# mathjeff/Mapper

Measured on NVIDIA B200. Metric: aligned reads/sec, higher is better.
Workload: dtype f64

## Files before the change

mapper_b200/csrc/xm_align.h:

```cpp
#pragma once
#include "xm_seed.h"

namespace xm {

struct Blk { int a_start, b_start, a_len, b_len; };
struct DAln {
  int valid, n;
  Blk* b;
  double penalty, aligned;
  int ref_reversed;
};
struct ACtx {
  SeqView a; int a_reversed_obj;
  SeqView b;
};
struct Sec { int start, end; XM_INLINE int length() const { return end - start; } };

struct MatcherD {
  int ref_start, ref_len, block_len, section_len, max_section_index;
  int loc_size;
  uint32_t* materialized;
  int mat_words;
  int16_t* tables; int table_entries, n_slots, slots_used;
  int slot_section[8];
};
static const int16_t T_NO = -1, T_MULTI = -2;
struct Analysis {
  MatcherD* matcher;
  int predicted, last_checked, confident;
  double max_ins, max_del;
};

XM_INLINE DAln aln_null() { DAln a; a.valid = 0; a.n = 0; a.b = nullptr; a.penalty = 0; a.aligned = 0; a.ref_reversed = 0; return a; }

XM_FN double block_penalty(const Params& p, const ACtx& c, const Blk& k) {
  double pen = 0;
  if (k.a_len == k.b_len) {
#if defined(__CUDA_ARCH__)
    const int lane = (int)(threadIdx.x & 31);
    XM_NOUNROLL
    for (int base = 0; base < k.a_len; base += 32) {
      const int i = base + lane;
      double v = 0;
      if (i < k.a_len) v = p.base_penalty(c.a.at(k.a_start + i), c.b.at(k.b_start + i));
      unsigned m = __ballot_sync(0xffffffffu, v != 0);
      XM_NOUNROLL
      while (m) { const int src = __ffs(m) - 1; m &= m - 1; pen += __shfl_sync(0xffffffffu, v, src); }
    }
    __syncwarp();
#else
    XM_NOUNROLL
    for (int i = 0; i < k.a_len; i++) pen += p.base_penalty(c.a.at(k.a_start + i), c.b.at(k.b_start + i));
#endif
  } else if (k.a_len > 0) { pen += p.ins_start; pen += p.ins_ext * k.a_len; }
  else { pen += p.del_start; pen += p.del_ext * k.b_len; }
  return pen;
}
XM_FN double block_penalty_range(const Params& p, const SeqView& a, const SeqView& b, const Blk& k, int start_b, int end_b) {
  double pen = 0;
  if (k.a_len == k.b_len) {
#if defined(__CUDA_ARCH__)
    const int lane = (int)(threadIdx.x & 31);
    XM_NOUNROLL
    for (int base = 0; base < k.a_len; base += 32) {
      const int i = base + lane, bi = k.b_start + i;
      double v = 0;
      if (i < k.a_len && bi >= start_b && bi < end_b) v = p.base_penalty(a.at(k.a_start + i), b.at(bi));
      unsigned m = __ballot_sync(0xffffffffu, v != 0);
      XM_NOUNROLL
      while (m) { const int src = __ffs(m) - 1; m &= m - 1; pen += __shfl_sync(0xffffffffu, v, src); }
    }
    __syncwarp();
#else
    XM_NOUNROLL
    for (int i = 0; i < k.a_len; i++) { int bi = k.b_start + i; if (bi >= start_b && bi < end_b) pen += p.base_penalty(a.at(k.a_start + i), b.at(bi)); }
#endif
  } else if (k.b_start < end_b && k.b_start + k.b_len > start_b) {
    if (k.a_len > 0) { pen += p.ins_start; pen += p.ins_ext * k.a_len; } else { pen += p.del_start; pen += p.del_ext * k.b_len; }
  }
  return pen;
}
XM_FN DAln new_aln(const Params& p, const ACtx& c, Blk* blocks, int n, int ref_reversed) {
  int aligned_len = 0;
  double total = 0;
  XM_NOUNROLL
  for (int i = 0; i < n; i++) { total += block_penalty(p, c, blocks[i]); aligned_len += blocks[i].a_len; }
  if (n > 0 && p.start_free && blocks[0].b_len == 0) total -= p.ins_start;
  double aligned = total;
  if (n > 0) { int un = c.a.len - aligned_len; total += (double)un * p.unaligned; }
  DAln r; r.valid = 1; r.n = n; r.b = blocks; r.penalty = total; r.aligned = aligned; r.ref_reversed = ref_reversed;
  return r;
}
XM_INLINE int aln_start_a(const DAln& a) { return a.b[0].a_start; }
XM_INLINE int aln_end_a(const DAln& a) { return a.b[a.n - 1].a_start + a.b[a.n - 1].a_len; }
XM_INLINE int aln_start_b(const DAln& a) { return a.b[0].b_start; }
XM_INLINE int aln_end_b(const DAln& a) { return a.b[a.n - 1].b_start + a.b[a.n - 1].b_len; }

static const int M_NO = -1, M_MULTI = -2, M_UNKNOWN = -3;

XM_HD inline int log4_floor_plus1(int x) {
  int k = 0; long long p = 4;
  XM_NOUNROLL
  while (p <= (long long)x) { k++; p *= 4; }
  return k + 1;
}
XM_FN MatcherD* matcher_new(WS& w, const ACtx& c, const Sec& rsec, int section_len) {
  MatcherD* m = (MatcherD*)w.salloc(sizeof(MatcherD));
  if (!m) return nullptr;
  if (section_len < 1) section_len = 1;
  m->block_len = log4_floor_plus1(section_len * 5);
  if (m->block_len < 3) m->block_len = 3;
  m->ref_start = rsec.start; m->ref_len = rsec.length(); m->section_len = section_len;
  m->max_section_index = (c.b.len - 1 - m->ref_start) / section_len;
  m->loc_size = 0;
  int n_sec = imin(m->max_section_index + 1, (m->ref_len + 1) / section_len + 2);
  int words = (n_sec + 31) / 32;
  if (words < 1) words = 1;
  if (words > 4096) words = 4096;
  m->mat_words = words;
  m->materialized = (uint32_t*)w.salloc((long long)words * 4);
  if (!m->materialized) return nullptr;
  XM_NOUNROLL
  for (int i = 0; i < words; i++) m->materialized[i] = 0;
  m->tables = nullptr; m->table_entries = 0; m->n_slots = 0; m->slots_used = 0;
  if (section_len >= 3 && section_len < 32000 && m->block_len <= 7) {
    int entries = 1 << (2 * m->block_len);
    int slots = imin(8, m->max_section_index + 1);
    long long bytes = (long long)slots * entries * 2 + 16;
    if (slots > 0 && w.scratch_top + bytes + 4096 <= w.scratch_size / 2) {
      char* p = (char*)w.salloc(bytes);
      p += (16 - ((uintptr_t)p & 15)) & 15;
      m->tables = (int16_t*)p; m->table_entries = entries; m->n_slots = slots;
    }
  }
  return m;
}
XM_HD inline int matcher_encode(const SeqView& s, int index, int block_len) {
  if (index + block_len > s.len) return M_UNKNOWN;
  int sum = 0;
  XM_NOUNROLL
  for (int i = 0; i < block_len; i++) {
    uint8_t h = s.at(index + i);
    if (bp_is_ambiguous(h)) return M_UNKNOWN;
    sum = sum * 4 + (h == 1 ? 0 : h == 2 ? 1 : h == 4 ? 2 : 3);
  }
  return sum;
}
template <class F>
XM_INLINE void matcher_scan_encodings(const MatcherD& m, const SeqView& ref, int section_index, F&& f) {
  int max_poss = (1 << (2 * m.block_len)) - 1;
  int prev = M_UNKNOWN;
  int start = m.ref_start + section_index * m.section_len;
  int end = imin(start + m.section_len, m.ref_start + m.ref_len - m.block_len);
  XM_NOUNROLL
  for (int i = start; i < end; i++) {
    int enc;
    if (prev == M_UNKNOWN) enc = matcher_encode(ref, i, m.block_len);
    else {
      uint8_t nc = ref.at(i + m.block_len - 1);
      if (bp_is_ambiguous(nc)) enc = M_UNKNOWN;
      else enc = ((prev * 4) & max_poss) + (nc == 1 ? 0 : nc == 2 ? 1 : nc == 4 ? 2 : 3);
    }
    if (enc == M_UNKNOWN) continue;
    f(i - start, enc);
    prev = enc;
  }
}
XM_FN int matcher_section_value(WS& w, MatcherD& m, const SeqView& ref, int section_index, int target) {
  XM_CHECK_MASK(w);
  int start = m.ref_start + section_index * m.section_len;
  if (m.tables != nullptr) {
    int slot = -1;
    XM_NOUNROLL
    for (int i = 0; i < m.slots_used; i++) if (m.slot_section[i] == section_index) { slot = i; break; }
    if (slot < 0 && m.slots_used < m.n_slots) {
      PhaseClock pc_(&w.st_cyc[4]);
      slot = m.slots_used++;
      m.slot_section[slot] = section_index;
      int16_t* t = m.tables + (long long)slot * m.table_entries;
#if defined(__CUDA_ARCH__)
      {
        uint4 fill = make_uint4(0xFFFFFFFFu, 0xFFFFFFFFu, 0xFFFFFFFFu, 0xFFFFFFFFu);
        uint4* t4 = (uint4*)t;
        int n16 = m.table_entries / 8;
        XM_NOUNROLL
        for (int i = (int)(threadIdx.x & 31); i < n16; i += 32) t4[i] = fill;
        __syncwarp();
      }
#else
      XM_NOUNROLL
      for (int i = 0; i < m.table_entries; i++) t[i] = T_NO;
#endif
      matcher_scan_encodings(m, ref, section_index, [&](int rel, int enc) { t[enc] = (t[enc] == T_NO) ? (int16_t)rel : T_MULTI; });
    }
    if (slot >= 0) {
      int16_t v = m.tables[(long long)slot * m.table_entries + target];
      return v == T_NO ? M_NO : v == T_MULTI ? M_MULTI : start + (int)v;
    }
  }
  int value = M_NO;
  matcher_scan_encodings(m, ref, section_index, [&](int rel, int enc) { if (enc == target) value = (value == M_NO) ? start + rel : M_MULTI; });
  return value;
}
XM_HD inline bool matcher_get_section(WS& w, MatcherD& m, int index) {
  if (index >= m.mat_words * 32) { w.fail(Q_NEED_MORE); return false; }
  if (m.loc_size > index) return (m.materialized[index >> 5] >> (index & 31)) & 1;
  m.loc_size = index + 1;
  m.materialized[index >> 5] |= (1u << (index & 31));
  return true;
}
XM_FN int matcher_scan_section(const MatcherD& m, const ACtx& c, int query_index, int section_index) {
  int result = M_NO;
  int start = m.ref_start + section_index * m.section_len, end = start + m.section_len;
  XM_NOUNROLL
  for (int i = start; i < end; i++) {
    bool ok = !(i + m.block_len > m.ref_start + m.ref_len);
    XM_NOUNROLL
    for (int k = 0; ok && k < m.block_len; k++) {
      if (query_index + k >= c.a.len || i + k >= c.b.len) { ok = false; break; }
      if (!bp_can_match(c.a.at(query_index + k), c.b.at(i + k))) ok = false;
    }
    if (ok) { if (result == M_NO) result = i; else return M_MULTI; }
  }
  return result;
}
XM_FN int matcher_lookup(WS& w, MatcherD& m, const ACtx& c, int query_index, int min_ref, int max_ref) {
  XM_CHECK_MASK(w);
  if (min_ref < 0) return M_UNKNOWN;
  if (max_ref > c.b.len) return M_UNKNOWN;
  int enc = matcher_encode(c.a, query_index, m.block_len);
  if (enc < 0) return M_UNKNOWN;
  int matched = M_NO;
  int min_sec = imax(0, (min_ref - m.ref_start) / m.section_len);
  int max_sec = imin(m.max_section_index, (max_ref - m.ref_start) / m.section_len);
  XM_NOUNROLL
  for (int si = min_sec; si <= max_sec; si++) {
    bool have = matcher_get_section(w, m, si);
    if (w.status != 0) return M_UNKNOWN;
    int looked;
    if (m.section_len < 3) looked = matcher_scan_section(m, c, query_index, si);
    else { if (have) looked = matcher_section_value(w, m, c.b, si, enc); else return M_UNKNOWN; }
    if (looked == M_UNKNOWN) return M_UNKNOWN;
    if (looked == M_MULTI) return M_MULTI;
    if (looked == M_NO) continue;
    if (looked < min_ref || looked > max_ref) continue;
    if (matched != M_NO) return M_MULTI;
    matched = looked;
  }
  return matched;
}

struct alignas(16) PNode { double pen, ins_x, ins_y; uint32_t stamp; uint32_t meta; };
struct alignas(8) PMeta { uint32_t stamp, meta; };
struct PEnt { uint32_t xy; int32_t next; };
struct PathState {
  Params prm; ACtx ctx;
  int an_confident; double an_max_ins, an_max_del;
  int start_a, end_a, start_b, end_b, A, B, W, H;
  int diagonal, step, reverse, may_extend;
  int start_x, start_y, goal_x, goal_y;
  PNode* nodes; uint32_t gen; uint32_t clock;
  const uint8_t* qa; const uint8_t* rb;
  PEnt* ent; int ent_cap;
  double max_interesting;
};
XM_INLINE uint8_t pa_qa(const PathState& s, int i) { return s.qa[i]; }
XM_INLINE uint8_t pa_rb(const PathState& s, int j) { return s.rb[j]; }
XM_INLINE bool pa_can_remove(const Blk& b) {
  if (b.a_len <= 0 && b.b_len <= 0) return true;
  if ((b.a_start <= 0 && b.a_len <= 0) || (b.b_start <= 0 && b.b_len <= 0)) return true;
  return false;
}
XM_INLINE uint32_t pa_pack_xy(int x, int y) { return ((uint32_t)(uint16_t)(int16_t)x << 16) | (uint32_t)(uint16_t)(int16_t)y; }

struct PaOverflow { double key; int head, tail; };
struct PaQueue {
  PEnt* ent; int n_ent, cap, free_head;
  double cur_key; int cur_head, cur_tail;
  PaOverflow* ovf; int ovf_lo, ovf_hi, cap_ovf;
#if defined(__CUDA_ARCH__)
  double bkey; int bhead, btail;
#else
  double bkey[32]; int bhead[32], btail[32];
#endif
  XM_INLINE void init(PEnt* e, int capacity, PaOverflow* o, int cap_o) {
    ent = e; n_ent = 0; cap = capacity; free_head = -1; cur_key = 0; cur_head = -1; cur_tail = -1; ovf = o; ovf_lo = 0; ovf_hi = 0; cap_ovf = cap_o;
#if defined(__CUDA_ARCH__)
    bkey = 0; bhead = -1; btail = -1;
#else
    for (int i = 0; i < 32; i++) { bkey[i] = 0; bhead[i] = -1; btail[i] = -1; }
#endif
  }
  XM_INLINE int push(double pri, int x, int y) {
    int id;
    if (n_ent < cap) id = n_ent++;
    else { if (free_head < 0) return 1; id = free_head; free_head = ent[id].next; }
    PEnt e; e.xy = pa_pack_xy(x, y); e.next = -1;
    ent[id] = e;
    if (pri == cur_key) {
      if (cur_tail >= 0) ent[cur_tail].next = id; else cur_head = id;
      cur_tail = id;
      return 0;
    }
#if defined(__CUDA_ARCH__)
    const int lane = (int)(threadIdx.x & 31);
    const unsigned hit = __ballot_sync(0xffffffffu, bhead >= 0 && bkey == pri);
    if (hit != 0) {
      const int b = __ffs(hit) - 1;
      const int t = __shfl_sync(0xffffffffu, btail, b);
      ent[t].next = id;
      if (lane == b) btail = id;
      return 0;
    }
#else
    for (int b = 0; b < 32; b++) if (bhead[b] >= 0 && bkey[b] == pri) { ent[btail[b]].next = id; btail[b] = id; return 0; }
#endif
    int lo = ovf_lo, hi = ovf_hi;
#if defined(__CUDA_ARCH__)
    XM_NOUNROLL
    while (hi - lo > 0) {
      const int n = hi - lo;
      const int stride = (n + 31) >> 5;
      const int at = lo + imin(n, (lane + 1) * stride) - 1;
      const bool less = ovf[at].key < pri;
      const int k = __popc(__ballot_sync(0xffffffffu, less));
      const int nlo = lo + imin(n, k * stride);
      if (k >= 32 || nlo >= hi) { lo = hi; break; }
      hi = lo + imin(n, (k + 1) * stride); lo = nlo;
      if (stride == 1) { break; }
    }
#else
    XM_NOUNROLL
    while (lo < hi) { const int mid = (lo + hi) >> 1; if (ovf[mid].key < pri) lo = mid + 1; else hi = mid; }
#endif
    if (lo < ovf_hi && ovf[lo].key == pri) { ent[ovf[lo].tail].next = id; ovf[lo].tail = id; return 0; }
#if defined(__CUDA_ARCH__)
    const unsigned fre = __ballot_sync(0xffffffffu, bhead < 0);
    if (fre != 0) { const int b = __ffs(fre) - 1; if (lane == b) { bkey = pri; bhead = id; btail = id; } return 0; }
#else
    for (int b = 0; b < 32; b++) if (bhead[b] < 0) { bkey[b] = pri; bhead[b] = id; btail[b] = id; return 0; }
#endif
    if (ovf_hi >= cap_ovf) {
      if (ovf_lo == 0) return 2;
      const int n = ovf_hi - ovf_lo;
#if defined(__CUDA_ARCH__)
      XM_NOUNROLL
      for (int base = 0; base < n; base += 32) {
        const int i = base + lane;
        PaOverflow t; if (i < n) t = ovf[ovf_lo + i];
        __syncwarp();
        if (i < n) ovf[i] = t;
        __syncwarp();
      }
#else
      for (int i = 0; i < n; i++) ovf[i] = ovf[ovf_lo + i];
#endif
      lo -= ovf_lo; ovf_lo = 0; ovf_hi = n;
    }
    {
#if defined(__CUDA_ARCH__)
      XM_NOUNROLL
      for (int top = ovf_hi; top > lo; top -= 32) {
        const int i = top - 1 - lane;
        PaOverflow t; if (i >= lo) t = ovf[i];
        __syncwarp();
        if (i >= lo) ovf[i + 1] = t;
        __syncwarp();
      }
#else
      for (int i = ovf_hi - 1; i >= lo; i--) ovf[i + 1] = ovf[i];
#endif
      PaOverflow t; t.key = pri; t.head = id; t.tail = id;
      ovf[lo] = t;
      ovf_hi++;
    }
    return 0;
  }
  XM_INLINE bool pop(int& x, int& y) {
    if (cur_head < 0) {
      bool have = false; double best = 0; int where = -1;
#if defined(__CUDA_ARCH__)
      const int lane = (int)(threadIdx.x & 31);
      const unsigned live = __ballot_sync(0xffffffffu, bhead >= 0);
      if (live != 0) {
        const unsigned long long bits = (unsigned long long)__double_as_longlong(bkey);
        const unsigned hi = bhead >= 0 ? (unsigned)(bits >> 32) : 0xffffffffu;
        const unsigned mhi = __reduce_min_sync(0xffffffffu, hi);
        const unsigned lo = (bhead >= 0 && hi == mhi) ? (unsigned)bits : 0xffffffffu;
        const unsigned mlo = __reduce_min_sync(0xffffffffu, lo);
        const unsigned who = __ballot_sync(0xffffffffu, bhead >= 0 && hi == mhi && (unsigned)bits == mlo);
        where = __ffs(who) - 1;
        best = __longlong_as_double((long long)(((unsigned long long)mhi << 32) | mlo));
        have = true;
      }
#else
      for (int b = 0; b < 32; b++) if (bhead[b] >= 0 && (!have || bkey[b] < best)) { have = true; best = bkey[b]; where = b; }
#endif
      if (ovf_lo < ovf_hi && (!have || ovf[ovf_lo].key < best)) { have = true; best = ovf[ovf_lo].key; where = 32; }
      if (!have) return false;
      cur_key = best;
      if (where >= 32) { cur_head = ovf[ovf_lo].head; cur_tail = ovf[ovf_lo].tail; ovf_lo++; if (ovf_lo == ovf_hi) { ovf_lo = 0; ovf_hi = 0; } }
      else {
#if defined(__CUDA_ARCH__)
        cur_head = __shfl_sync(0xffffffffu, bhead, where); cur_tail = __shfl_sync(0xffffffffu, btail, where);
        if (lane == where) bhead = -1;
#else
        cur_head = bhead[where]; cur_tail = btail[where]; bhead[where] = -1;
#endif
      }
    }
    const PEnt e = ent[cur_head];
    ent[cur_head].next = free_head; free_head = cur_head;
    cur_head = e.next;
    if (cur_head < 0) cur_tail = -1;
    x = (int)(int16_t)(e.xy >> 16); y = (int)(int16_t)(e.xy & 0xffffu);
    return true;
  }
};

XM_INLINE int pa_signed_dist(const PathState& s, int x, int y) { return x - y - s.diagonal; }
XM_INLINE PNode pa_node(const PathState& s, int idx) {
#if defined(__CUDA_ARCH__)
  const double2 a = __ldcg((const double2*)&s.nodes[idx]);
  const double2 b = __ldcg((const double2*)&s.nodes[idx] + 1);
  PNode n; n.pen = a.x; n.ins_x = a.y; n.ins_y = b.x;
  const unsigned long long m = (unsigned long long)__double_as_longlong(b.y);
  n.stamp = (uint32_t)m; n.meta = (uint32_t)(m >> 32);
  return n;
#else
  return s.nodes[idx];
#endif
}
XM_INLINE bool pa_get(const PathState& s, int x, int y, int& idx) {
  if (x < 0 || x >= s.W || y < 0 || y >= s.H) return false;
  idx = x * s.H + y;
  return (pa_node(s, idx).meta >> 8) == s.gen;
}
XM_HD inline double pa_estimate(const PathState& s, int x, int y, const PNode& n, int fl) {
  if (!s.an_confident) return n.pen;
  int sd = pa_signed_dist(s, x, y);
  const Params& p = s.prm;
  if (fl & 2) {
    if (sd * s.step > 0) { double ie = fabs(sd * p.ins_ext); if (ie > s.an_max_ins) return XM_DISALLOWED; }
    else { double de = fabs(sd * p.del_ext); if (de > s.an_max_del) return XM_DISALLOWED; }
    if (fl & 4) return n.pen;
    return n.pen + dmin(p.ins_start + p.ins_ext, p.del_start + p.del_ext);
  }
  if (sd * s.step < 0) {
    double ie = fabs(sd * p.ins_ext);
    if (ie > s.an_max_ins) return XM_DISALLOWED;
    double is = dmin(p.ins_start, n.ins_x - n.pen);
    return n.pen + is + ie;
  } else {
    double de = fabs(sd * p.del_ext);
    if (de > s.an_max_del) return XM_DISALLOWED;
    double ds = dmin(p.del_start, n.ins_y - n.pen);
    return n.pen + ds + de;
  }
}
XM_FN int pa_search(WS& w, PathState& S, PaOverflow* ovf, int cap_ovf, int& last_x, int& last_y) {
  XM_CHECK_MASK(w);
  const int A = S.A, B = S.B, H = S.H, step = S.step, goal_x = S.goal_x, goal_y = S.goal_y, diag = S.diagonal;
  const bool may_extend = S.may_extend != 0, confident = S.an_confident != 0;
  const double ins_start = S.prm.ins_start, ins_ext = S.prm.ins_ext, del_start = S.prm.del_start, del_ext = S.prm.del_ext, unaligned = S.prm.unaligned;
  const double max_ins = S.an_max_ins, max_del = S.an_max_del, budget = S.max_interesting + 0.000001;
  const double min_indel = dmin(ins_start + ins_ext, del_start + del_ext);
  const double* pen_tab = S.prm.pen_tab; const uint8_t* cls_tab = S.prm.cls_tab;
  PNode* nodes = S.nodes; const uint8_t* qa = S.qa; const uint8_t* rb = S.rb;
  const uint32_t gen = S.gen; const int W = S.W;
  uint32_t clock = S.clock;
  PaQueue Q;
  Q.init(S.ent, S.ent_cap, ovf, cap_ovf);
  int qrc = 0;
  {
    const int start_x = S.start_x, start_y = S.start_y;
    const bool along_y = B >= A;
    double sisp = XM_DISALLOWED;
    if (along_y && may_extend) sisp = S.prm.starting_ins_start();
    const int cnt1 = (along_y ? imax(0, B - A) : imax(0, A - B)) + 1;
    const int cnt2 = may_extend ? imax(0, j2i(S.an_max_ins / del_ext) - 1) : 0;
    XM_NOUNROLL
    for (int i = 0; i < cnt1 + cnt2 && qrc == 0; i++) {
      PNode n; int x, y;
      if (i < cnt1) {
        n.pen = 0; n.ins_x = along_y ? sisp : XM_DISALLOWED; n.ins_y = XM_DISALLOWED;
        x = along_y ? start_x : start_x + i * step; y = along_y ? start_y + i * step : start_y;
      } else {
        const int k = i - cnt1 + 1;
        x = start_x + k * step; y = start_y;
        n.pen = k * unaligned; n.ins_x = XM_DISALLOWED; n.ins_y = XM_DISALLOWED;
        if (x < -32000 || x > 32000) { qrc = 1; break; }
      }
      n.stamp = ++clock; n.meta = gen << 8;
      qrc = Q.push(pa_estimate(S, x, y, n, 0), x, y);
      if (x >= 0 && x < W) nodes[x * H + y] = n;
    }
  }
  unsigned long long steps = 0;
  int rc = 2;
  XM_NOUNROLL
  while (qrc == 0) {
    int tx, ty;
    if (!Q.pop(tx, ty)) { w.fail(Q_INTERNAL); break; }
    const double active = Q.cur_key;
    steps++;
    if (active > budget) { rc = 1; break; }
    if (tx == goal_x) { last_x = tx; last_y = ty; rc = 0; break; }
    XM_NOUNROLL
    for (int nb = 0; nb < 3; nb++) {
      const int x = tx + (nb != 1 ? step : 0), y = ty + (nb != 0 ? step : 0);
      if (x <= 0 || x > A || y <= 0 || y > B) continue;
      const int ie = x * H + y, il = ie - step * H, iu = ie - step, id = il - step;
      const PMeta me = *(const PMeta*)&nodes[ie].stamp, ml = *(const PMeta*)&nodes[il].stamp, mu = *(const PMeta*)&nodes[iu].stamp, md = *(const PMeta*)&nodes[id].stamp;
      const bool he = (me.meta >> 8) == gen, hl = (ml.meta >> 8) == gen, hu = (mu.meta >> 8) == gen, hd = (md.meta >> 8) == gen;
      if (he) {
        uint32_t newest = 0;
        if (hl && ml.stamp > newest) newest = ml.stamp;
        if (hu && mu.stamp > newest) newest = mu.stamp;
        if (hd && md.stamp > newest) newest = md.stamp;
        if (me.stamp > newest) continue;
      }
      const uint32_t fl_ = hl ? (1u | (ml.meta & 6u)) : 0u, fu = hu ? (1u | (mu.meta & 6u)) : 0u, fd = hd ? (1u | (md.meta & 6u)) : 0u;
      double ins_x = XM_DISALLOWED, ins_y = XM_DISALLOWED, overlay = XM_DISALLOWED;
      if (hd) overlay = nodes[id].pen + pen_tab[((int)qa[x - 1] << 4) | (int)rb[y - 1]];
      if (hl) {
        const double lp = nodes[il].pen;
        if (y == goal_y && may_extend) ins_x = lp + unaligned;
        else {
          bool allowed = (cls_tab[((int)qa[x - 1 - step] << 5) | (int)rb[y - 1]] & 1) != 0;
          if (allowed) allowed = (cls_tab[((int)qa[x - 1] << 5) | (int)rb[y - 1 + step]] & 6) == 0;
          const double nw = allowed ? lp + ins_start + ins_ext : XM_DISALLOWED;
          ins_x = dmin(nodes[il].ins_x + ins_ext, nw);
        }
      }
      if (hu) {
        bool allowed = (cls_tab[((int)qa[x - 1] << 5) | (int)rb[y - 1 - step]] & 1) != 0;
        if (allowed) allowed = (cls_tab[((int)qa[x - 1 + step] << 5) | (int)rb[y - 1]] & 6) == 0;
        const double nw = allowed ? nodes[iu].pen + del_start + del_ext : XM_DISALLOWED;
        ins_y = dmin(nodes[iu].ins_y + del_ext, nw);
      }
      const double best = dmin(dmin(overlay, ins_x), ins_y);
      if (he && !(best < nodes[ie].pen || ins_x < nodes[ie].ins_x || ins_y < nodes[ie].ins_y)) continue;
      const int sd = x - y - diag;
      int fl = 0;
      if (best != XM_DISALLOWED) {
        const int src = (best == overlay) ? fd : (best == ins_x) ? fl_ : fu;
        fl = (src & 6) | (sd == 0 ? 2 : 4);
      }
      double est = best;
      if (confident) {
        const int sds = sd * step;
        if (fl & 2) {
          const bool over = (sds > 0) ? (fabs(sd * ins_ext) > max_ins) : (fabs(sd * del_ext) > max_del);
          if (over) est = XM_DISALLOWED;
          else if (!(fl & 4)) est = best + min_indel;
        } else if (sds < 0) {
          const double ie_ = fabs(sd * ins_ext);
          if (ie_ > max_ins) est = XM_DISALLOWED;
          else est = best + dmin(ins_start, ins_x - best) + ie_;
        } else {
          const double de = fabs(sd * del_ext);
          if (de > max_del) est = XM_DISALLOWED;
          else est = best + dmin(del_start, ins_y - best) + de;
        }
      }
      if (est < active) est = active;
      qrc = Q.push(est, x, y);
      if (qrc != 0) break;
      PNode n; n.pen = best; n.ins_x = ins_x; n.ins_y = ins_y; n.stamp = ++clock; n.meta = (gen << 8) | (uint32_t)fl;
      nodes[ie] = n;
    }
  }
  S.clock = clock;
  if (qrc != 0) { w.fail(Q_NEED_MORE); rc = 2; }
  w.st_path_steps += steps;
  return rc;
}

XM_FN DAln path_align(WS& w, const ACtx& c, const Sec& q, const Sec& r, const Params& p, Analysis& an) {
  XM_CHECK_MASK(w);
  PhaseClock pc_(&w.st_cyc[3]);
  long long mark = w.scratch_top;
  PathState* sp = (PathState*)w.salloc(sizeof(PathState));
  if (!sp) return aln_null();
  PathState& s = *sp;
  s.prm = p; s.ctx = c; s.an_confident = an.confident; s.an_max_ins = an.max_ins; s.an_max_del = an.max_del;
  s.max_interesting = q.length() * p.max_error_rate;
  s.start_a = q.start; s.end_a = q.end; s.start_b = r.start; s.end_b = r.end;
  s.A = q.length(); s.B = r.length(); s.W = s.A + 2; s.H = s.B + 2;
  s.diagonal = s.start_b - (s.start_a + an.predicted);
  {
    uint8_t* qa = (uint8_t*)w.salloc(s.A + 5); uint8_t* rb = (uint8_t*)w.salloc(s.B + 5);
    if (w.status != 0) { w.scratch_top = mark; return aln_null(); }
    qa += 2; rb += 2;
    XM_NOUNROLL
    for (int k = 0; k < 2; k++) { qa[-1 - k] = 16; qa[s.A + k] = 16; rb[-1 - k] = 16; rb[s.B + k] = 16; }
#if defined(__CUDA_ARCH__)
    for (int k = (int)(threadIdx.x & 31); k < s.A; k += 32) qa[k] = c.a.at(s.start_a + k);
    for (int k = (int)(threadIdx.x & 31); k < s.B; k += 32) rb[k] = c.b.at(s.start_b + k);
    __syncwarp();
#else
    for (int k = 0; k < s.A; k++) qa[k] = c.a.at(s.start_a + k);
    for (int k = 0; k < s.B; k++) rb[k] = c.b.at(s.start_b + k);
#endif
    s.qa = qa; s.rb = rb;
  }
  w.st_path_calls++; w.st_path_cells += (unsigned long long)s.A * (unsigned long long)s.B;
  {
    int sum_mis = 0, num_mis = 0, sum_mat = 0, num_mat = 0;
    int si = imax(s.start_a, s.start_b - an.predicted), ei = imin(s.end_a, s.end_b - an.predicted);
    int length = ei - si;
#if defined(__CUDA_ARCH__)
    XM_NOUNROLL
    for (int i = (int)(threadIdx.x & 31); i < length; i += 32) {
      int j = i - s.diagonal;
      if (j >= 0 && j < s.B) {
        if (!bp_can_match(pa_qa(s, i), pa_rb(s, j))) { sum_mis += i; num_mis++; } else { sum_mat += i; num_mat++; }
      }
    }
    __syncwarp();
    sum_mis = __reduce_add_sync(0xffffffffu, sum_mis); num_mis = __reduce_add_sync(0xffffffffu, num_mis);
    sum_mat = __reduce_add_sync(0xffffffffu, sum_mat); num_mat = __reduce_add_sync(0xffffffffu, num_mat);
#else
    XM_NOUNROLL
    for (int i = 0; i < length; i++) {
      int j = i - s.diagonal;
      if (j >= 0 && j < s.B) {
        if (!bp_can_match(pa_qa(s, i), pa_rb(s, j))) { sum_mis += i; num_mis++; } else { sum_mat += i; num_mat++; }
      }
    }
#endif
    s.reverse = (num_mis > 1 && num_mat > 1) ? ((sum_mis / num_mis) > (sum_mat / num_mat) ? 1 : 0) : 1;
  }
  if (s.reverse) { s.step = -1; s.may_extend = (s.start_b == 0); } else { s.step = 1; s.may_extend = (s.end_b == c.b.len); }
  if (s.reverse) { s.start_x = s.W - 1; s.start_y = s.H - 1; s.goal_x = 1; s.goal_y = 1; }
  else { s.start_x = 0; s.start_y = 0; s.goal_x = s.W - 2; s.goal_y = s.H - 2; }
  long long cells = (long long)s.W * (long long)s.H;
  if (s.W > 32000 || s.H > 32000) { w.fail(Q_NEED_MORE); w.scratch_top = mark; return aln_null(); }
  const long long map_words = cells * (long long)(sizeof(PNode) / 4);
  if (w.cell_hdr == nullptr || map_words > w.cell_words) { w.fail(Q_NEED_MORE); w.scratch_top = mark; return aln_null(); }
  {
    uint32_t gen = w.cell_hdr[0];
    if (gen == 0 || gen >= 0xFFFFFF) {
      const long long n16 = (w.cell_words + 3) >> 2;
#if defined(__CUDA_ARCH__)
      uint4* c4 = (uint4*)w.cellmap;
      XM_NOUNROLL
      for (long long i = (long long)(threadIdx.x & 31); i < n16; i += 32) c4[i] = make_uint4(0u, 0u, 0u, 0u);
      __syncwarp();
#else
      for (long long i = 0; i < w.cell_words; i++) w.cellmap[i] = 0;
#endif
      gen = 0;
    }
    gen++;
#if defined(__CUDA_ARCH__)
    if ((threadIdx.x & 31) == 0) w.cell_hdr[0] = gen;
    __syncwarp();
#else
    w.cell_hdr[0] = gen;
#endif
    s.nodes = (PNode*)w.cellmap; s.gen = gen; s.clock = 0;
  }
  long long remaining = w.scratch_size - w.scratch_top;
  int cap_ovf = (int)(s.max_interesting * 64.0) + 256;
  if ((long long)cap_ovf * (long long)sizeof(PaOverflow) > remaining / 8) cap_ovf = (int)((remaining / 8) / (long long)sizeof(PaOverflow));
  PaOverflow* ovf = (PaOverflow*)w.salloc((long long)cap_ovf * (long long)sizeof(PaOverflow));
  long long ent_cap = (remaining / 2) / (long long)sizeof(PEnt);
  if (ent_cap > 3 * cells + 64) ent_cap = 3 * cells + 64;
  s.ent_cap = (int)ent_cap;
  s.ent = (PEnt*)w.salloc(ent_cap * (long long)sizeof(PEnt));
  if (w.status != 0 || s.ent_cap < 8) { w.fail(Q_NEED_MORE); w.scratch_top = mark; return aln_null(); }
  int last_x = -1, last_y = -1;
  {
    const int rc = pa_search(w, s, ovf, cap_ovf, last_x, last_y);
    if (rc == 1 && w.status == 0) { w.scratch_top = mark; return aln_null(); }
  }
  if (w.status != 0) { w.scratch_top = mark; return aln_null(); }
  int max_blocks = s.A + s.B + 4;
  Blk* tb = (Blk*)w.salloc((long long)max_blocks * (long long)sizeof(Blk));
  if (!tb) { w.scratch_top = mark; return aln_null(); }
  int nb = 0;
  int i = last_x, j = last_y, idx;
  XM_NOUNROLL
  while (i != s.start_x && j != s.start_y) {
    if (!pa_get(s, i, j, idx)) { w.fail(Q_INTERNAL); break; }
    PNode node = pa_node(s, idx);
    Blk k;
    if (node.pen == node.ins_x) {
      int old_i = i;
      i -= s.step;
      XM_NOUNROLL
      while (i != s.start_x) {
        if (!pa_get(s, i, j, idx)) { w.fail(Q_INTERNAL); break; }
        const PNode o = pa_node(s, idx);
        if (o.pen + p.ins_start + p.ins_ext < o.ins_x + p.ins_ext) break;
        i -= s.step;
      }
      if (s.reverse) { k.a_start = s.start_a + old_i - 1; k.b_start = s.start_b + j - 1; k.a_len = i - old_i; k.b_len = 0; }
      else { k.a_start = s.start_a + i; k.b_start = s.start_b + j; k.a_len = old_i - i; k.b_len = 0; }
    } else if (node.pen == node.ins_y) {
      int old_j = j;
      j -= s.step;
      XM_NOUNROLL
      while (j != s.start_y) {
        if (!pa_get(s, i, j, idx)) { w.fail(Q_INTERNAL); break; }
        const PNode o = pa_node(s, idx);
        if (o.pen + p.del_start + p.del_ext < o.ins_y + p.del_ext) break;
        j -= s.step;
      }
      if (s.reverse) { k.a_start = s.start_a + i - 1; k.b_start = s.start_b + old_j - 1; k.a_len = 0; k.b_len = j - old_j; }
      else { k.a_start = s.start_a + i; k.b_start = s.start_b + j; k.a_len = 0; k.b_len = old_j - j; }
    } else {
      int old_i = i, old_j = j;
      i -= s.step; j -= s.step;
      XM_NOUNROLL
      while (i != s.start_x && j != s.start_y) {
        if (!pa_get(s, i, j, idx)) { w.fail(Q_INTERNAL); break; }
        const PNode o = pa_node(s, idx);
        if (o.pen == o.ins_x || o.pen == o.ins_y) break;
        i -= s.step; j -= s.step;
      }
      if (s.reverse) { k.a_start = s.start_a + old_i - 1; k.b_start = s.start_b + old_j - 1; k.a_len = i - old_i; k.b_len = j - old_j; }
      else { k.a_start = s.start_a + i; k.b_start = s.start_b + j; k.a_len = old_i - i; k.b_len = old_j - j; }
    }
    if (w.status != 0) break;
    if (nb >= max_blocks) { w.fail(Q_INTERNAL); break; }
    tb[nb++] = k;
  }
  if (w.status != 0) { w.scratch_top = mark; return aln_null(); }
  if (!s.reverse) { for (int a = 0, b = nb - 1; a < b; a++, b--) { Blk t = tb[a]; tb[a] = tb[b]; tb[b] = t; } }
  if (nb < 1) { w.scratch_top = mark; return aln_null(); }
  XM_NOUNROLL
  for (int m = 1; m < nb - 1; m++) {
    XM_NOUNROLL
    while (true) {
      Blk left = tb[m - 1], mid = tb[m], right = tb[m + 1];
      if ((mid.a_len > 0) == (mid.b_len > 0)) break;
      if (left.a_len == 0 || left.b_len == 0) break;
      if (right.a_len == 0 || right.b_len == 0) break;
      if (mid.a_len > 0) { if (c.a.at(left.a_start + left.a_len - 1) != c.a.at(mid.a_start + mid.a_len - 1)) break; }
      else { if (c.b.at(left.b_start + left.b_len - 1) != c.b.at(mid.b_start + mid.b_len - 1)) break; }
      left.a_len -= 1; left.b_len -= 1;
      mid.a_start -= 1; mid.b_start -= 1;
      right.a_start -= 1; right.b_start -= 1; right.a_len += 1; right.b_len += 1;
      tb[m - 1] = left; tb[m] = mid; tb[m + 1] = right;
    }
  }
  int first = 0;
  XM_NOUNROLL
  while (true) {
    if (first >= nb) { w.fail(Q_INTERNAL); w.scratch_top = mark; return aln_null(); }
    if (!pa_can_remove(tb[first])) break;
    first++;
  }
  int n_out = nb - first;
  double max_int = s.max_interesting;
  w.scratch_top = mark;
  Blk* out = (Blk*)w.salloc((long long)n_out * (long long)sizeof(Blk));
  XM_NOUNROLL
  for (int a = 0; a < n_out; a++) out[a] = tb[first + a];
  DAln res = new_aln(p, c, out, n_out, c.a_reversed_obj);
  if (res.aligned > max_int) { w.scratch_top = mark; return aln_null(); }
  return res;
}

enum { ST_STRAIGHT1 = 0, ST_SKIP = 1, ST_HBA1 = 2, ST_BLOCK = 3, ST_STRAIGHT2 = 4, ST_HBA2 = 5, ST_STRAIGHT3 = 6, ST_PATH = 7 };
template <int STAGE>
XM_HD DAln cascade_t(WS& w, const ACtx& c, const Sec& q, const Sec& r, const Params& p, Analysis& an);

XM_HD inline DAln straight_alignment(WS& w, const ACtx& c, const Sec& q, const Sec& r, const Params& p, const Analysis& an) {
  int qs = q.start, qe = q.end, rs = r.start, re = r.end, off = an.predicted;
  if (qs + off > rs) rs = qs + off; else qs = rs - off;
  if (qe + off < re) re = qe + off; else qe = re - off;
  Blk* b = (Blk*)w.salloc(sizeof(Blk));
  if (!b) return aln_null();
  b->a_start = qs; b->b_start = rs; b->a_len = qe - qs; b->b_len = re - rs;
  return new_aln(p, c, b, 1, c.a_reversed_obj);
}
template <bool EASY, int STAGE>
XM_FN DAln straight_align_t(WS& w, const ACtx& c, const Sec& q, const Sec& r, const Params& p, Analysis& an) {
  XM_CHECK_MASK(w);
  an.last_checked = an.predicted;
  w.st_straight++;
  DAln simple;
  { PhaseClock pc_(&w.st_cyc[1]); simple = straight_alignment(w, c, q, r, p, an); }
  if (!simple.valid) return simple;
  double sp = simple.aligned;
  double max_interesting = q.length() * p.max_error_rate;
  double indel = dmin(p.starting_ins_start() + p.ins_ext, p.del_start + p.del_ext);
  if (sp <= 0) return simple;
  if (an.confident) {
    if (sp <= indel || (an.max_ins <= 0 && an.max_del <= 0)) { if (sp <= max_interesting) return simple; return aln_null(); }
    if (indel > max_interesting) return aln_null();
  }
  double rate = simple.aligned / q.length();
  Params sub = p;
  sub.max_error_rate = dmin(rate, p.max_error_rate);
  if constexpr (EASY) { w.hard_hint = (int)(sp * 16.0); w.fail(Q_HARD); return aln_null(); }
  else {
    DAln a = cascade_t<STAGE + 1>(w, c, q, r, sub, an);
    if (w.status != 0) return aln_null();
    if (!a.valid || a.aligned >= sp) { if (sp <= max_interesting) return simple; }
    return a;
  }
}

struct CountMapD {
  int most_key, most_count, have;
  int* keys; int* vals; int n, cap;
};
XM_HD inline void countmap_put(WS& w, CountMapD& m, int key, int val) {
  XM_NOUNROLL
  for (int i = 0; i < m.n; i++) if (m.keys[i] == key) { m.vals[i] = val; return; }
  if (m.n >= m.cap) { w.fail(Q_NEED_MORE); return; }
  m.keys[m.n] = key; m.vals[m.n] = val; m.n++;
}
XM_FN void countmap_add(WS& w, CountMapD& m, int key, int value) {
  if (key == m.most_key || m.most_count == 0) {
    m.most_count += value; m.most_key = key;
    if (m.have) countmap_put(w, m, m.most_key, m.most_count);
  } else {
    if (!m.have) { m.have = 1; countmap_put(w, m, m.most_key, m.most_count); }
    int count = value;
    XM_NOUNROLL
    for (int i = 0; i < m.n; i++) if (m.keys[i] == key) { count = m.vals[i] + value; break; }
    countmap_put(w, m, key, count);
    if (count > m.most_count) { m.most_key = key; m.most_count = count; }
  }
}

XM_HD inline double min_indel_penalty_for_block_mismatches(int n, const Params& p) {
  n = imax(1, n);
  double per_initial = dmin(p.starting_ins_start() + p.ins_ext, p.del_start + p.del_ext);
  double per_ext = dmin(p.ins_ext, p.del_ext);
  double per_subseq_indel = dmin(p.ins_start + p.ins_ext, p.del_start + p.del_ext);
  double per_subseq = dmin(p.mutation, per_subseq_indel);
  if (n <= 1) return per_initial;
  if (n <= 2) return per_initial + per_ext;
  return per_initial + per_ext + (n - 2) * per_subseq;
}
XM_HD inline double max_ext_long_insertion(int n, double total, const Params& p, int block_len) {
  double avail = total - p.starting_ins_start();
  double only_snps = n * p.mutation;
  double per_block = block_len * p.ins_ext;
  double extra_per_block = per_block - p.mutation;
  if (extra_per_block <= 0) return avail;
  if (n < 2) return avail;
  double short_ext = 2 * p.ins_ext;
  if (short_ext > avail) return avail;
  double short_snps = 2 * p.mutation;
  double past = avail - only_snps;
  double for_blocks = past + short_snps - short_ext;
  double num = for_blocks / extra_per_block;
  double r = (num * block_len + 2) * p.ins_ext;
  r = dmin(r, avail);
  if (r < short_ext) r = 0;
  return r;
}
XM_HD inline double max_ext_many_insertions(int n, double total, const Params& p) {
  double avail = total + (p.ins_start - p.starting_ins_start());
  double only_snps = n * p.mutation;
  double per_short = p.ins_start + 2 * p.ins_ext;
  double extra = per_short - 2 * p.mutation;
  if (extra <= 0) return avail;
  double num = (avail - only_snps) / extra;
  if (num < 1) num = 0;
  double r = num * 2 * p.ins_ext;
  return dmin(r, avail);
}
XM_HD inline double max_ext_many_deletions(int n, double total, const Params& p) {
  double avail = total;
  double only_snps = n * p.mutation;
  double per_short = p.del_start + 2 * p.del_ext;
  double extra = per_short - 2 * p.mutation;
  if (extra <= 0) return avail;
  double num = (avail - only_snps) / extra;
  if (num < 1) num = 0;
// ... 1022 lines not shown
```

Measured before the change: 2.337 million.

## Move path-search loop state into a per-warp shared-memory frame

The A* path search loop and its priority queue now keep their invariants and queue bookkeeping in a per-warp `PaFrame` in static shared memory, instead of in registers. Values are re-read through volatile loads at each use so the compiler cannot cache them in registers. The goal is to cut register pressure and spills in the large alignment kernel and so raise occupancy. In exchange, many register reads become shared-memory loads on the hot loop, and the node write and clock increment now happen before the queue push.

```diff
diff --git a/mapper_b200/csrc/xm_align.h b/mapper_b200/csrc/xm_align.h
--- a/mapper_b200/csrc/xm_align.h
+++ b/mapper_b200/csrc/xm_align.h
@@ -274,32 +274,54 @@
 XM_INLINE uint32_t pa_pack_xy(int x, int y) { return ((uint32_t)(uint16_t)(int16_t)x << 16) | (uint32_t)(uint16_t)(int16_t)y; }
 
 struct PaOverflow { double key; int head, tail; };
+struct PaFrame {
+  const double* pen_tab; const uint8_t* cls_tab; PNode* nodes; const uint8_t* qa; const uint8_t* rb;
+  double ins_start, ins_ext, del_start, del_ext, unaligned, max_ins, max_del, budget, min_indel;
+  unsigned long long steps;
+  PEnt* ent; PaOverflow* ovf;
+  double cur_key;
+  int n_ent, cap, free_head, cur_head, cur_tail, ovf_lo, ovf_hi, cap_ovf;
+  int A, B, H, step, goal_x, goal_y, diagonal;
+  uint32_t gen, clock;
+  int16_t tx, ty, x, y;
+  uint8_t may_extend, confident;
+};
+static_assert(sizeof(PaFrame) == 224, "32 frames keep the full kernel's static shared memory within 48 KB");
+template <class T> XM_INLINE T pa_ld(const T& v) {
+#if defined(__CUDA_ARCH__)
+  return *(const volatile T*)&v;
+#else
+  return v;
+#endif
+}
+#if defined(__CUDA_ARCH__)
+__shared__ PaFrame pa_frame[32];
+#endif
 struct PaQueue {
-  PEnt* ent; int n_ent, cap, free_head;
-  double cur_key; int cur_head, cur_tail;
-  PaOverflow* ovf; int ovf_lo, ovf_hi, cap_ovf;
 #if defined(__CUDA_ARCH__)
   double bkey; int bhead, btail;
 #else
   double bkey[32]; int bhead[32], btail[32];
 #endif
-  XM_INLINE void init(PEnt* e, int capacity, PaOverflow* o, int cap_o) {
-    ent = e; n_ent = 0; cap = capacity; free_head = -1; cur_key = 0; cur_head = -1; cur_tail = -1; ovf = o; ovf_lo = 0; ovf_hi = 0; cap_ovf = cap_o;
+  XM_INLINE void init(PaFrame& f, PEnt* e, int capacity, PaOverflow* o, int cap_o) {
+    f.ent = e; f.n_ent = 0; f.cap = capacity; f.free_head = -1; f.cur_key = 0; f.cur_head = -1; f.cur_tail = -1; f.ovf = o; f.ovf_lo = 0; f.ovf_hi = 0; f.cap_ovf = cap_o;
 #if defined(__CUDA_ARCH__)
     bkey = 0; bhead = -1; btail = -1;
 #else
     for (int i = 0; i < 32; i++) { bkey[i] = 0; bhead[i] = -1; btail[i] = -1; }
 #endif
   }
-  XM_INLINE int push(double pri, int x, int y) {
+  XM_INLINE int push(PaFrame& f, double pri, int x, int y) {
+    PEnt* const ent = f.ent;
     int id;
-    if (n_ent < cap) id = n_ent++;
-    else { if (free_head < 0) return 1; id = free_head; free_head = ent[id].next; }
+    if (f.n_ent < f.cap) { id = f.n_ent; f.n_ent = id + 1; }
+    else { id = f.free_head; if (id < 0) return 1; f.free_head = ent[id].next; }
     PEnt e; e.xy = pa_pack_xy(x, y); e.next = -1;
     ent[id] = e;
-    if (pri == cur_key) {
-      if (cur_tail >= 0) ent[cur_tail].next = id; else cur_head = id;
-      cur_tail = id;
+    if (pri == f.cur_key) {
+      const int t = f.cur_tail;
+      if (t >= 0) ent[t].next = id; else f.cur_head = id;
+      f.cur_tail = id;
       return 0;
     }
 #if defined(__CUDA_ARCH__)
@@ -315,7 +337,8 @@
 #else
     for (int b = 0; b < 32; b++) if (bhead[b] >= 0 && bkey[b] == pri) { ent[btail[b]].next = id; btail[b] = id; return 0; }
 #endif
-    int lo = ovf_lo, hi = ovf_hi;
+    PaOverflow* const ovf = f.ovf;
+    int lo = f.ovf_lo, hi = f.ovf_hi;
 #if defined(__CUDA_ARCH__)
     XM_NOUNROLL
     while (hi - lo > 0) {
@@ -333,34 +356,36 @@
     XM_NOUNROLL
     while (lo < hi) { const int mid = (lo + hi) >> 1; if (ovf[mid].key < pri) lo = mid + 1; else hi = mid; }
 #endif
-    if (lo < ovf_hi && ovf[lo].key == pri) { ent[ovf[lo].tail].next = id; ovf[lo].tail = id; return 0; }
+    if (lo < f.ovf_hi && ovf[lo].key == pri) { ent[ovf[lo].tail].next = id; ovf[lo].tail = id; return 0; }
 #if defined(__CUDA_ARCH__)
     const unsigned fre = __ballot_sync(0xffffffffu, bhead < 0);
     if (fre != 0) { const int b = __ffs(fre) - 1; if (lane == b) { bkey = pri; bhead = id; btail = id; } return 0; }
 #else
     for (int b = 0; b < 32; b++) if (bhead[b] < 0) { bkey[b] = pri; bhead[b] = id; btail[b] = id; return 0; }
 #endif
-    if (ovf_hi >= cap_ovf) {
-      if (ovf_lo == 0) return 2;
-      const int n = ovf_hi - ovf_lo;
+    if (f.ovf_hi >= f.cap_ovf) {
+      const int olo = f.ovf_lo;
+      if (olo == 0) return 2;
+      const int n = f.ovf_hi - olo;
 #if defined(__CUDA_ARCH__)
       XM_NOUNROLL
       for (int base = 0; base < n; base += 32) {
         const int i = base + lane;
-        PaOverflow t; if (i < n) t = ovf[ovf_lo + i];
+        PaOverflow t; if (i < n) t = ovf[olo + i];
         __syncwarp();
         if (i < n) ovf[i] = t;
         __syncwarp();
       }
 #else
-      for (int i = 0; i < n; i++) ovf[i] = ovf[ovf_lo + i];
-#endif
-      lo -= ovf_lo; ovf_lo = 0; ovf_hi = n;
+      for (int i = 0; i < n; i++) ovf[i] = ovf[olo + i];
+#endif
+      lo -= olo; f.ovf_lo = 0; f.ovf_hi = n;
     }
     {
-#if defined(__CUDA_ARCH__)
-      XM_NOUNROLL
-      for (int top = ovf_hi; top > lo; top -= 32) {
+      const int ohi = f.ovf_hi;
+#if defined(__CUDA_ARCH__)
+      XM_NOUNROLL
+      for (int top = ohi; top > lo; top -= 32) {
         const int i = top - 1 - lane;
         PaOverflow t; if (i >= lo) t = ovf[i];
         __syncwarp();
@@ -368,16 +393,18 @@
         __syncwarp();
       }
 #else
-      for (int i = ovf_hi - 1; i >= lo; i--) ovf[i + 1] = ovf[i];
+      for (int i = ohi - 1; i >= lo; i--) ovf[i + 1] = ovf[i];
 #endif
       PaOverflow t; t.key = pri; t.head = id; t.tail = id;
       ovf[lo] = t;
-      ovf_hi++;
+      f.ovf_hi = ohi + 1;
     }
     return 0;
   }
-  XM_INLINE bool pop(int& x, int& y) {
-    if (cur_head < 0) {
+  XM_INLINE bool pop(PaFrame& f, int& x, int& y) {
+    PEnt* const ent = f.ent;
+    int head = f.cur_head;
+    if (head < 0) {
       bool have = false; double best = 0; int where = -1;
 #if defined(__CUDA_ARCH__)
       const int lane = (int)(threadIdx.x & 31);
@@ -396,23 +423,27 @@
 #else
       for (int b = 0; b < 32; b++) if (bhead[b] >= 0 && (!have || bkey[b] < best)) { have = true; best = bkey[b]; where = b; }
 #endif
-      if (ovf_lo < ovf_hi && (!have || ovf[ovf_lo].key < best)) { have = true; best = ovf[ovf_lo].key; where = 32; }
+      const int olo = f.ovf_lo;
+      if (olo < f.ovf_hi && (!have || f.ovf[olo].key < best)) { have = true; best = f.ovf[olo].key; where = 32; }
       if (!have) return false;
-      cur_key = best;
-      if (where >= 32) { cur_head = ovf[ovf_lo].head; cur_tail = ovf[ovf_lo].tail; ovf_lo++; if (ovf_lo == ovf_hi) { ovf_lo = 0; ovf_hi = 0; } }
-      else {
-#if defined(__CUDA_ARCH__)
-        cur_head = __shfl_sync(0xffffffffu, bhead, where); cur_tail = __shfl_sync(0xffffffffu, btail, where);
+      f.cur_key = best;
+      if (where >= 32) {
+        const PaOverflow o = f.ovf[olo];
+        head = o.head; f.cur_tail = o.tail;
+        if (olo + 1 == f.ovf_hi) { f.ovf_lo = 0; f.ovf_hi = 0; } else f.ovf_lo = olo + 1;
+      } else {
+#if defined(__CUDA_ARCH__)
+        head = __shfl_sync(0xffffffffu, bhead, where); f.cur_tail = __shfl_sync(0xffffffffu, btail, where);
         if (lane == where) bhead = -1;
 #else
-        cur_head = bhead[where]; cur_tail = btail[where]; bhead[where] = -1;
-#endif
-      }
-    }
-    const PEnt e = ent[cur_head];
-    ent[cur_head].next = free_head; free_head = cur_head;
-    cur_head = e.next;
-    if (cur_head < 0) cur_tail = -1;
+        head = bhead[where]; f.cur_tail = btail[where]; bhead[where] = -1;
+#endif
+      }
+    }
+    const PEnt e = ent[head];
+    ent[head].next = f.free_head; f.free_head = head;
+    f.cur_head = e.next;
+    if (e.next < 0) f.cur_tail = -1;
     x = (int)(int16_t)(e.xy >> 16); y = (int)(int16_t)(e.xy & 0xffffu);
     return true;
   }
@@ -460,25 +491,28 @@
 }
 XM_FN int pa_search(WS& w, PathState& S, PaOverflow* ovf, int cap_ovf, int& last_x, int& last_y) {
   XM_CHECK_MASK(w);
-  const int A = S.A, B = S.B, H = S.H, step = S.step, goal_x = S.goal_x, goal_y = S.goal_y, diag = S.diagonal;
-  const bool may_extend = S.may_extend != 0, confident = S.an_confident != 0;
-  const double ins_start = S.prm.ins_start, ins_ext = S.prm.ins_ext, del_start = S.prm.del_start, del_ext = S.prm.del_ext, unaligned = S.prm.unaligned;
-  const double max_ins = S.an_max_ins, max_del = S.an_max_del, budget = S.max_interesting + 0.000001;
-  const double min_indel = dmin(ins_start + ins_ext, del_start + del_ext);
-  const double* pen_tab = S.prm.pen_tab; const uint8_t* cls_tab = S.prm.cls_tab;
-  PNode* nodes = S.nodes; const uint8_t* qa = S.qa; const uint8_t* rb = S.rb;
-  const uint32_t gen = S.gen; const int W = S.W;
-  uint32_t clock = S.clock;
+#if defined(__CUDA_ARCH__)
+  PaFrame& F = pa_frame[threadIdx.x >> 5];
+#else
+  PaFrame frame; PaFrame& F = frame;
+#endif
+  F.A = S.A; F.B = S.B; F.H = S.H; F.step = S.step; F.goal_x = S.goal_x; F.goal_y = S.goal_y; F.diagonal = S.diagonal;
+  F.may_extend = S.may_extend != 0; F.confident = S.an_confident != 0;
+  F.ins_start = S.prm.ins_start; F.ins_ext = S.prm.ins_ext; F.del_start = S.prm.del_start; F.del_ext = S.prm.del_ext; F.unaligned = S.prm.unaligned;
+  F.max_ins = S.an_max_ins; F.max_del = S.an_max_del; F.budget = S.max_interesting + 0.000001;
+  F.min_indel = dmin(S.prm.ins_start + S.prm.ins_ext, S.prm.del_start + S.prm.del_ext);
+  F.pen_tab = S.prm.pen_tab; F.cls_tab = S.prm.cls_tab; F.nodes = S.nodes; F.qa = S.qa; F.rb = S.rb;
+  F.gen = S.gen; F.clock = S.clock; F.steps = 0;
   PaQueue Q;
-  Q.init(S.ent, S.ent_cap, ovf, cap_ovf);
+  Q.init(F, S.ent, S.ent_cap, ovf, cap_ovf);
   int qrc = 0;
   {
-    const int start_x = S.start_x, start_y = S.start_y;
-    const bool along_y = B >= A;
+    const int A = S.A, B = S.B, step = S.step, start_x = S.start_x, start_y = S.start_y;
+    const bool along_y = B >= A, may_extend = S.may_extend != 0;
     double sisp = XM_DISALLOWED;
     if (along_y && may_extend) sisp = S.prm.starting_ins_start();
     const int cnt1 = (along_y ? imax(0, B - A) : imax(0, A - B)) + 1;
-    const int cnt2 = may_extend ? imax(0, j2i(S.an_max_ins / del_ext) - 1) : 0;
+    const int cnt2 = may_extend ? imax(0, j2i(S.an_max_ins / S.prm.del_ext) - 1) : 0;
     XM_NOUNROLL
     for (int i = 0; i < cnt1 + cnt2 && qrc == 0; i++) {
       PNode n; int x, y;
@@ -488,92 +522,119 @@
       } else {
         const int k = i - cnt1 + 1;
         x = start_x + k * step; y = start_y;
-        n.pen = k * unaligned; n.ins_x = XM_DISALLOWED; n.ins_y = XM_DISALLOWED;
+        n.pen = k * S.prm.unaligned; n.ins_x = XM_DISALLOWED; n.ins_y = XM_DISALLOWED;
         if (x < -32000 || x > 32000) { qrc = 1; break; }
       }
-      n.stamp = ++clock; n.meta = gen << 8;
-      qrc = Q.push(pa_estimate(S, x, y, n, 0), x, y);
-      if (x >= 0 && x < W) nodes[x * H + y] = n;
-    }
-  }
-  unsigned long long steps = 0;
+      const uint32_t clock = F.clock + 1;
+      F.clock = clock;
+      n.stamp = clock; n.meta = S.gen << 8;
+      qrc = Q.push(F, pa_estimate(S, x, y, n, 0), x, y);
+      if (x >= 0 && x < S.W) S.nodes[x * S.H + y] = n;
+    }
+  }
   int rc = 2;
   XM_NOUNROLL
   while (qrc == 0) {
-    int tx, ty;
-    if (!Q.pop(tx, ty)) { w.fail(Q_INTERNAL); break; }
-    const double active = Q.cur_key;
-    steps++;
-    if (active > budget) { rc = 1; break; }
-    if (tx == goal_x) { last_x = tx; last_y = ty; rc = 0; break; }
+    {
+      int tx, ty;
+      if (!Q.pop(F, tx, ty)) { w.fail(Q_INTERNAL); break; }
+      F.tx = (int16_t)tx; F.ty = (int16_t)ty;
+      F.steps = F.steps + 1;
+      if (F.cur_key > F.budget) { rc = 1; break; }
+      if (tx == F.goal_x) { last_x = tx; last_y = ty; rc = 0; break; }
+    }
     XM_NOUNROLL
     for (int nb = 0; nb < 3; nb++) {
-      const int x = tx + (nb != 1 ? step : 0), y = ty + (nb != 0 ? step : 0);
-      if (x <= 0 || x > A || y <= 0 || y > B) continue;
-      const int ie = x * H + y, il = ie - step * H, iu = ie - step, id = il - step;
-      const PMeta me = *(const PMeta*)&nodes[ie].stamp, ml = *(const PMeta*)&nodes[il].stamp, mu = *(const PMeta*)&nodes[iu].stamp, md = *(const PMeta*)&nodes[id].stamp;
-      const bool he = (me.meta >> 8) == gen, hl = (ml.meta >> 8) == gen, hu = (mu.meta >> 8) == gen, hd = (md.meta >> 8) == gen;
+      {
+        const int step = pa_ld(F.step);
+        const int x = pa_ld(F.tx) + (nb != 1 ? step : 0), y = pa_ld(F.ty) + (nb != 0 ? step : 0);
+        if (x <= 0 || x > pa_ld(F.A) || y <= 0 || y > pa_ld(F.B)) continue;
+        F.x = (int16_t)x; F.y = (int16_t)y;
+      }
+      uint32_t fpk;
+      bool he;
+      {
+        PNode* const nodes = pa_ld(F.nodes);
+        const int step = pa_ld(F.step), ie = pa_ld(F.x) * pa_ld(F.H) + pa_ld(F.y), il = ie - step * pa_ld(F.H), iu = ie - step, id = il - step;
+        const PMeta me = *(const PMeta*)&nodes[ie].stamp, ml = *(const PMeta*)&nodes[il].stamp, mu = *(const PMeta*)&nodes[iu].stamp, md = *(const PMeta*)&nodes[id].stamp;
+        const uint32_t gen = pa_ld(F.gen);
+        he = (me.meta >> 8) == gen;
+        const bool hl = (ml.meta >> 8) == gen, hu = (mu.meta >> 8) == gen, hd = (md.meta >> 8) == gen;
+        if (he) {
+          uint32_t newest = 0;
+          if (hl && ml.stamp > newest) newest = ml.stamp;
+          if (hu && mu.stamp > newest) newest = mu.stamp;
+          if (hd && md.stamp > newest) newest = md.stamp;
+          if (me.stamp > newest) continue;
+        }
+        fpk = (hd ? (1u | (md.meta & 6u)) : 0u) | (hl ? (1u | (ml.meta & 6u)) << 3 : 0u) | (hu ? (1u | (mu.meta & 6u)) << 6 : 0u);
+      }
+      double ins_x = XM_DISALLOWED, ins_y = XM_DISALLOWED, overlay = XM_DISALLOWED;
+      {
+        PNode* const nodes = pa_ld(F.nodes);
+        const uint8_t* const qa = pa_ld(F.qa); const uint8_t* const rb = pa_ld(F.rb); const uint8_t* const cls_tab = pa_ld(F.cls_tab);
+        const int x = pa_ld(F.x), y = pa_ld(F.y), step = pa_ld(F.step), ie = x * pa_ld(F.H) + y;
+        if (fpk & 1u) overlay = nodes[ie - step * pa_ld(F.H) - step].pen + pa_ld(F.pen_tab)[((int)qa[x - 1] << 4) | (int)rb[y - 1]];
+        if (fpk & 8u) {
+          const int il = ie - step * pa_ld(F.H);
+          const double lp = nodes[il].pen;
+          if (y == pa_ld(F.goal_y) && pa_ld(F.may_extend)) ins_x = lp + pa_ld(F.unaligned);
+          else {
+            bool allowed = (cls_tab[((int)qa[x - 1 - step] << 5) | (int)rb[y - 1]] & 1) != 0;
+            if (allowed) allowed = (cls_tab[((int)qa[x - 1] << 5) | (int)rb[y - 1 + step]] & 6) == 0;
+            const double nw = allowed ? lp + pa_ld(F.ins_start) + pa_ld(F.ins_ext) : XM_DISALLOWED;
+            ins_x = dmin(nodes[il].ins_x + pa_ld(F.ins_ext), nw);
+          }
+        }
+        if (fpk & 64u) {
+          const int iu = ie - step;
+          bool allowed = (cls_tab[((int)qa[x - 1] << 5) | (int)rb[y - 1 - step]] & 1) != 0;
+          if (allowed) allowed = (cls_tab[((int)qa[x - 1 + step] << 5) | (int)rb[y - 1]] & 6) == 0;
+          const double nw = allowed ? nodes[iu].pen + pa_ld(F.del_start) + pa_ld(F.del_ext) : XM_DISALLOWED;
+          ins_y = dmin(nodes[iu].ins_y + pa_ld(F.del_ext), nw);
+        }
+      }
+      const double best = dmin(dmin(overlay, ins_x), ins_y);
       if (he) {
-        uint32_t newest = 0;
-        if (hl && ml.stamp > newest) newest = ml.stamp;
-        if (hu && mu.stamp > newest) newest = mu.stamp;
-        if (hd && md.stamp > newest) newest = md.stamp;
-        if (me.stamp > newest) continue;
-      }
-      const uint32_t fl_ = hl ? (1u | (ml.meta & 6u)) : 0u, fu = hu ? (1u | (mu.meta & 6u)) : 0u, fd = hd ? (1u | (md.meta & 6u)) : 0u;
-      double ins_x = XM_DISALLOWED, ins_y = XM_DISALLOWED, overlay = XM_DISALLOWED;
-      if (hd) overlay = nodes[id].pen + pen_tab[((int)qa[x - 1] << 4) | (int)rb[y - 1]];
-      if (hl) {
-        const double lp = nodes[il].pen;
-        if (y == goal_y && may_extend) ins_x = lp + unaligned;
-        else {
-          bool allowed = (cls_tab[((int)qa[x - 1 - step] << 5) | (int)rb[y - 1]] & 1) != 0;
-          if (allowed) allowed = (cls_tab[((int)qa[x - 1] << 5) | (int)rb[y - 1 + step]] & 6) == 0;
-          const double nw = allowed ? lp + ins_start + ins_ext : XM_DISALLOWED;
-          ins_x = dmin(nodes[il].ins_x + ins_ext, nw);
-        }
-      }
-      if (hu) {
-        bool allowed = (cls_tab[((int)qa[x - 1] << 5) | (int)rb[y - 1 - step]] & 1) != 0;
-        if (allowed) allowed = (cls_tab[((int)qa[x - 1 + step] << 5) | (int)rb[y - 1]] & 6) == 0;
-        const double nw = allowed ? nodes[iu].pen + del_start + del_ext : XM_DISALLOWED;
-        ins_y = dmin(nodes[iu].ins_y + del_ext, nw);
-      }
-      const double best = dmin(dmin(overlay, ins_x), ins_y);
-      if (he && !(best < nodes[ie].pen || ins_x < nodes[ie].ins_x || ins_y < nodes[ie].ins_y)) continue;
-      const int sd = x - y - diag;
+        const PNode* const o = pa_ld(F.nodes) + (pa_ld(F.x) * pa_ld(F.H) + pa_ld(F.y));
+        if (!(best < o->pen || ins_x < o->ins_x || ins_y < o->ins_y)) continue;
+      }
+      const int sd = pa_ld(F.x) - pa_ld(F.y) - pa_ld(F.diagonal);
       int fl = 0;
       if (best != XM_DISALLOWED) {
-        const int src = (best == overlay) ? fd : (best == ins_x) ? fl_ : fu;
-        fl = (src & 6) | (sd == 0 ? 2 : 4);
+        const uint32_t src = (best == overlay) ? fpk : (best == ins_x) ? fpk >> 3 : fpk >> 6;
+        fl = (int)(src & 6u) | (sd == 0 ? 2 : 4);
       }
       double est = best;
-      if (confident) {
-        const int sds = sd * step;
+      if (pa_ld(F.confident)) {
+        const int sds = sd * pa_ld(F.step);
         if (fl & 2) {
-          const bool over = (sds > 0) ? (fabs(sd * ins_ext) > max_ins) : (fabs(sd * del_ext) > max_del);
+          const bool over = (sds > 0) ? (fabs(sd * pa_ld(F.ins_ext)) > pa_ld(F.max_ins)) : (fabs(sd * pa_ld(F.del_ext)) > pa_ld(F.max_del));
           if (over) est = XM_DISALLOWED;
-          else if (!(fl & 4)) est = best + min_indel;
+          else if (!(fl & 4)) est = best + pa_ld(F.min_indel);
         } else if (sds < 0) {
-          const double ie_ = fabs(sd * ins_ext);
-          if (ie_ > max_ins) est = XM_DISALLOWED;
-          else est = best + dmin(ins_start, ins_x - best) + ie_;
+          const double ie_ = fabs(sd * pa_ld(F.ins_ext));
+          if (ie_ > pa_ld(F.max_ins)) est = XM_DISALLOWED;
+          else est = best + dmin(pa_ld(F.ins_start), ins_x - best) + ie_;
         } else {
-          const double de = fabs(sd * del_ext);
-          if (de > max_del) est = XM_DISALLOWED;
-          else est = best + dmin(del_start, ins_y - best) + de;
+          const double de = fabs(sd * pa_ld(F.del_ext));
+          if (de > pa_ld(F.max_del)) est = XM_DISALLOWED;
+          else est = best + dmin(pa_ld(F.del_start), ins_y - best) + de;
         }
       }
+      const uint32_t clock = pa_ld(F.clock) + 1;
+      F.clock = clock;
+      PNode n; n.pen = best; n.ins_x = ins_x; n.ins_y = ins_y; n.stamp = clock; n.meta = (pa_ld(F.gen) << 8) | (uint32_t)fl;
+      pa_ld(F.nodes)[(pa_ld(F.x) * pa_ld(F.H) + pa_ld(F.y))] = n;
+      const double active = pa_ld(F.cur_key);
       if (est < active) est = active;
-      qrc = Q.push(est, x, y);
+      qrc = Q.push(F, est, pa_ld(F.x), pa_ld(F.y));
       if (qrc != 0) break;
-      PNode n; n.pen = best; n.ins_x = ins_x; n.ins_y = ins_y; n.stamp = ++clock; n.meta = (gen << 8) | (uint32_t)fl;
-      nodes[ie] = n;
-    }
-  }
-  S.clock = clock;
+    }
+  }
+  S.clock = F.clock;
   if (qrc != 0) { w.fail(Q_NEED_MORE); rc = 2; }
-  w.st_path_steps += steps;
+  w.st_path_steps += F.steps;
   return rc;
 }
 
```

New measurement: 2.483 million (median of 6 runs). 1.06x the previous value.
